# Oliverbansk/Holistic-Robot-Pose-Estimation

Hardware: AMD Instinct MI355X
Metric: images/sec/GPU fwd+bwd HRNet-W32 256x256 bs=64; 1/2/4/8-GPU scaling (higher is better)
Workload: dtype bf16; 1 GPU; full network (HRNet-W32 reg backbone + HRNet-W32 DepthNet + heads + FK loss) fwd+loss+bwd+clip+Adam, BASELINE.json configs[2]; global_batch=64, per_gpu_batch=64, image=3x256x256, hrnet_w32_passes_per_image=2, parallelism=dp1, backend=single-process, rccl_ranks=1, hip_graph=True, plan_mode=hybrid, inputs=resident in HBM, optimizer=hrpe_amd.optim.FusedClipAdam (clip 5 + Adam, lr 1e-4)

## Files before the change

### holistic-robot-pose-estimation_amd/csrc/conv_batch.h

```cpp
#pragma once
#include "conv_row.h"
#include <string.h>

namespace hrp {

struct ConvProblem {
  hrp_conv_desc d;
  ConvTiling t;
  int cfg;
  int pgrid;
  int pad[2];
  RowPlan r;
};

template <typename T, int NT, bool LIGHT>
__global__ __launch_bounds__(256, LIGHT ? 1 : 2) void conv_batch_kernel(const ConvProblem* __restrict__ tab, const BatchHdr h) {
  int base;
  const int g = batch_find(h, blockIdx.x, base);
  const ConvProblem& P = tab[g];
  const int bid = (int)blockIdx.x - base;
  const int slot = blockIdx.x & (HRP_STAT_SLOTS - 1);
  if constexpr (LIGHT) {
    switch (P.cfg) {
      case 0: conv_tile_body<T, 1, 2, 1, 4, NT, false, true>(P.d, P.t, bid, 1, slot); break;
      case 1: conv_tile_body<T, 1, 1, 1, 4, NT, false, true>(P.d, P.t, bid, 1, slot); break;
      default:
        if constexpr (NT == 9) conv_tile_body<T, 1, 2, 1, 4, NT, true, true>(P.d, P.t, bid, P.pgrid, slot);
        break;
    }
  } else {
    switch (P.cfg) {
      case 0: conv_tile_body<T, 1, 2, 1, 4, NT, false, true>(P.d, P.t, bid, 1, slot); break;
      case 1: conv_tile_body<T, 1, 1, 1, 4, NT, false, true>(P.d, P.t, bid, 1, slot); break;
      case 2: conv_tile_body<T, 2, 2, 1, 4, NT, false, true>(P.d, P.t, bid, 1, slot); break;
      case 5: if constexpr (NT == 9 && Elem<T>::SZ == 2) conv_row_body<32>(P.d, P.r, bid, slot); break;
      case 6: if constexpr (NT == 9 && Elem<T>::SZ == 2) conv_row_body<64>(P.d, P.r, bid, slot); break;
      case 7: if constexpr (NT == 9 && Elem<T>::SZ == 2) conv_deep_body<128>(P.d, P.r, bid, slot); break;
      case 8: if constexpr (NT == 9 && Elem<T>::SZ == 2) conv_deep_body<256>(P.d, P.r, bid, slot); break;
      case 9: if constexpr (NT == 9 && Elem<T>::SZ == 2) conv_img_body<128>(P.d, P.r, bid, slot); break;
      case 10: if constexpr (NT == 9 && Elem<T>::SZ == 2) conv_img_body<256>(P.d, P.r, bid, slot); break;
      default: conv_tile_body<T, 2, 1, 1, 4, NT, false, true>(P.d, P.t, bid, 1, slot); break;
    }
  }
}

template <typename T, int NT>
static int conv_batch_plan_one(const hrp_conv_desc& d, ConvProblem& P, int& lds) {
  int rc = -100;
  if constexpr (NT == 9 && Elem<T>::SZ == 2) {
    const int rc_ = hrp_conv_rowstrip_channels(&d);
    if (rc_) {
      row_plan(d, P.r);
      P.t = ConvTiling{};
      P.t.nblocks = row_grid(P.r, rc_);
      P.cfg = rc_ == 32 ? 5 : rc_ == 64 ? 6 : rc_ == 128 ? 7 : 8;
      if (P.r.img) P.cfg += 2;
      lds = row_lds_bytes(rc_, P.r.img);
      return HRP_OK;
    }
  }
  static const int budget_kb = 76;
  g_conv_lds_budget_kb = budget_kb;
  if (d.Cout <= 32) {
    rc = plan_cfg<T, 1, 2, 1, 4, NT>(d, P.t, lds, false); P.cfg = 0;
    if (rc == -100) { rc = plan_cfg<T, 1, 1, 1, 4, NT>(d, P.t, lds, false); P.cfg = 1; }
  } else {
    rc = plan_cfg<T, 2, 2, 1, 4, NT>(d, P.t, lds, false); P.cfg = 2;
    if (rc == -100) { rc = plan_cfg<T, 2, 1, 1, 4, NT>(d, P.t, lds, false); P.cfg = 3; }
    if (rc == -100) { rc = plan_cfg<T, 1, 2, 1, 4, NT>(d, P.t, lds, false); P.cfg = 0; }
    if (rc == -100) { rc = plan_cfg<T, 1, 1, 1, 4, NT>(d, P.t, lds, false); P.cfg = 1; }
  }
  if (rc == -100) {
    set_error("conv batch: no tile configuration fits LDS and the tap halo (H=%d W=%d Cin=%d stride=%d taps=%d)", d.H, d.W, d.Cin, d.in_stride, d.ntaps);
    return HRP_ERR_ARG;
  }
  return rc;
}

template <typename T, int NT>
static int conv_batch_prepare_nt(const hrp_conv_desc* descs, int n, ConvProblem* tab, hrp_batch_info* info) {
  constexpr int SZ = Elem<T>::SZ;
  ConvProblem probs[HRP_BATCH_MAX];
  long weight[HRP_BATCH_MAX];
  int lds_max = 0;
  for (int i = 0; i < n; ++i) {
    const hrp_conv_desc& d = descs[i];
    HRP_REQUIRE((d.Cin * SZ) % ROW == 0, "conv batch: Cin * sizeof(T) must be a multiple of 32 bytes (Cin=%d)", d.Cin);
    memset(&probs[i], 0, sizeof(ConvProblem));
    probs[i].d = d;
    int lds = 0;
    const int rc = conv_batch_plan_one<T, NT>(d, probs[i], lds);
    if (rc != HRP_OK) return rc;
    lds_max = lds > lds_max ? lds : lds_max;
    const int ct = probs[i].cfg >= 2 ? 2 : 1, pt = (probs[i].cfg & 1) ? 1 : 2;
    weight[i] = (long)cdiv(d.Cin * SZ, ROW) * NT * ct * pt;
    if (probs[i].cfg >= 5) weight[i] = (long)cdiv(d.Cin * SZ, ROW) * NT * (probs[i].cfg == 9 ? 8 : 4);
  }
  int order[HRP_BATCH_MAX];
  for (int i = 0; i < n; ++i) order[i] = i;
  for (int i = 1; i < n; ++i)
    for (int j = i; j > 0 && weight[order[j]] > weight[order[j - 1]]; --j) { int t_ = order[j]; order[j] = order[j - 1]; order[j - 1] = t_; }
  bool light = true;
  for (int i = 0; i < n; ++i) light = light && probs[i].cfg <= 1;
  static const int pwgs = 512;
  const int pcap = light && pwgs > 0 ? (pwgs / n < 32 ? 32 : pwgs / n) : 0;
  int blk = 0;
  for (int k = 0; k < n; ++k) {
    ConvProblem& P = probs[order[k]];
    info->blk0[k] = blk;
    if (NT == 9 && pcap > 0 && P.cfg == 0 && P.t.nblocks >= 2 * pcap && P.d.Cin * SZ <= 2 * ROW && !P.d.bnb_x) {
      P.cfg = 4;
      P.pgrid = pcap;
      blk += pcap;
    } else {
      blk += P.t.nblocks;
    }
    if (tab) tab[k] = P;
  }
  info->blk0[n] = blk;
  info->grid = blk;
  info->lds_bytes = lds_max;
  info->variant = NT + (light ? 100 : 0);
  return HRP_OK;
}

template <typename T>
static int conv_batch_prepare_t(const hrp_conv_desc* descs, int n, void* table, hrp_batch_info* info) {
  for (int i = 0; i < n; ++i) {
    const int rc = conv_check(&descs[i]);
    if (rc != HRP_OK) return rc;
    HRP_REQUIRE(descs[i].ntaps == descs[0].ntaps && descs[i].dtype == descs[0].dtype, "conv batch: mixed tap counts / element types");
    HRP_REQUIRE(descs[i].ntaps != 1 || !descs[i].bnb_x || (descs[i].bnb_mask && descs[i].bnb_consts && !descs[i].res),
                "conv batch: a 1x1 problem with a mask-less / residual epilogue reduce must be launched on its own (hrp_conv_pointwise)");
    HRP_REQUIRE(!(descs[i].dtype == HRP_F32 && descs[i].H == 1 && descs[i].W == 1 && descs[i].Cin >= 512),
                "conv batch: linear layers are launched one by one");
  }
  ConvProblem* tab = (ConvProblem*)table;
  switch (descs[0].ntaps) {
    case 1: return conv_batch_prepare_nt<T, 1>(descs, n, tab, info);
    case 2: return conv_batch_prepare_nt<T, 2>(descs, n, tab, info);
    case 4: return conv_batch_prepare_nt<T, 4>(descs, n, tab, info);
    case 9: return conv_batch_prepare_nt<T, 9>(descs, n, tab, info);
    default:
      set_error("conv batch: ntaps=%d is not one of the batched tap counts (1, 2, 4, 9)", descs[0].ntaps);
      return HRP_ERR_ARG;
  }
}

template <typename T, int NT, bool LIGHT>
static int conv_batch_launch_nt(const void* table_dev, const hrp_batch_info* info, hipStream_t s) {
  static bool attr_set = false;
  if (!attr_set) {
    (void)hipFuncSetAttribute((const void*)conv_batch_kernel<T, NT, LIGHT>, hipFuncAttributeMaxDynamicSharedMemorySize, 160 * 1024);
    attr_set = true;
  }
  const BatchHdr h = make_hdr(info->blk0, info->n);
  hipLaunchKernelGGL((conv_batch_kernel<T, NT, LIGHT>), dim3(info->grid), dim3(256), info->lds_bytes, s, (const ConvProblem*)table_dev, h);
  return check_launch("conv_batch_kernel");
}

template <typename T>
static int conv_batch_launch_t(const void* table_dev, const hrp_batch_info* info, hipStream_t s) {
  switch (info->variant) {
    case 1: return conv_batch_launch_nt<T, 1, false>(table_dev, info, s);
    case 2: return conv_batch_launch_nt<T, 2, false>(table_dev, info, s);
    case 4: return conv_batch_launch_nt<T, 4, false>(table_dev, info, s);
    case 9: return conv_batch_launch_nt<T, 9, false>(table_dev, info, s);
    case 101: return conv_batch_launch_nt<T, 1, true>(table_dev, info, s);
    case 102: return conv_batch_launch_nt<T, 2, true>(table_dev, info, s);
    case 104: return conv_batch_launch_nt<T, 4, true>(table_dev, info, s);
    case 109: return conv_batch_launch_nt<T, 9, true>(table_dev, info, s);
    default: set_error("conv batch: bad variant %d", info->variant); return HRP_ERR_ARG;
  }
}

}
```

### holistic-robot-pose-estimation_amd/csrc/conv_row.h

```cpp
#pragma once
#include "conv_tile.h"
#include <type_traits>

namespace hrp {

template <int C>
struct RowCfg {
  static constexpr int W = 2048 / C;
  static constexpr int P = 2 * C;
  static constexpr int S = P / 16;
  static constexpr int KS = C / 16;
  static constexpr int MT = C / 32;
  static constexpr int NCOL = W / 32;
  static constexpr int TH = 8;
  static constexpr int PXP = 1024 / P;
  static constexpr int ROWB = (W + 1) * P;
  static constexpr int NROWS = TH + 2;
  static constexpr int TILE_BYTES = P + NROWS * ROWB;
  static constexpr int CTAB_OFF = (TILE_BYTES + 255) & ~255;
  static constexpr int STAT_OFF = CTAB_OFF + 10 * C * 4;
  static constexpr bool PERSIST = C == 32;
  static constexpr int WLDS_OFF = STAT_OFF + 4 * 64 * 4;
  static constexpr int LDS_BYTES = WLDS_OFF + (PERSIST ? 9 * KS * 1024 : 0);
  static_assert(MT * NCOL == 2, "two waves side by side (columns or channel tiles), two on top of each other");
  __device__ static __forceinline__ int g(int x) { return C == 32 ? (x >> 2) & 3 : (x >> 1) & 7; }
};

struct RowPlan {
  int wslot[9];
  int nstrips, spi;
  FastDiv fd_spi;
  int img;
  int spw;
};

__device__ __forceinline__ void row_bn_consts(const double* stats, const float* gamma, const float* beta, float count, float eps,
                                              int c, int C, float& mean, float& inv, float& sc, float& sh) {
  const float m = slot_sum(stats, c, 2 * C) / count;
  const float var = fmaxf(slot_sum(stats, C + c, 2 * C) / count - m * m, 0.f);
  inv = rsqrtf(var + eps);
  mean = m;
  sc = gamma[c] * inv;
  sh = beta[c] - m * sc;
}

__device__ __forceinline__ float row_bn_act(float x, float sc, float sh) { return fmaf(x, sc, sh); }

static inline int row_channels(const hrp_conv_desc& d) {
  if (d.dtype != HRP_BF16 || d.ntaps != 9 || d.in_stride != 1 || d.out_stride != 1) return 0;
  if (d.Cin != d.Cout || (d.Cin != 32 && d.Cin != 64 && d.Cin != 128 && d.Cin != 256)) return 0;
  const int C = d.Cin;
  if (d.W != 2048 / C || d.Wo != d.W || d.Ho != d.H || d.H % 8 || d.y_H != d.Ho || d.y_W != d.Wo) return 0;
  if (d.x_pitch != C || d.y_pitch != C || d.w_cout_pad != C || (d.res && d.res_pitch != C)) return 0;
  if (((uintptr_t)d.x | (uintptr_t)d.y | (uintptr_t)d.w | (uintptr_t)d.res) % 16) return 0;
  if (d.bias) return 0;
  if (d.bnb_x && (d.bnb_x_pitch != C || !d.bnb_stats || !d.bnb_gamma || !d.bnb_beta || !d.stats ||
                  d.relu || d.scale || (uintptr_t)d.bnb_x % 16)) return 0;
  if (d.bnb_x && d.bnb_mask && (d.bnb_mask_pitch != C / 8 || (uintptr_t)d.bnb_mask % 2)) return 0;
  if (d.pro_mode < 0 || d.pro_mode > 3) return 0;
  if (d.pro_mode && (!d.pro_stats || !d.pro_gamma || !d.pro_beta)) return 0;
  if (d.pro_mode == 2 && (!d.pro_x2 || !d.pro_bsums || (uintptr_t)d.pro_x2 % 16)) return 0;
  if (d.pro_mode == 3 && (!d.pro_x2 || (uintptr_t)d.pro_x2 % 16 || !d.pro_side || !d.pro_mask || d.pro_side2)) return 0;
  if (d.pro_mode < 2 && (d.pro_mask || d.pro_side2)) return 0;
  if ((d.pro_side && (uintptr_t)d.pro_side % 16) || (d.pro_side2 && (uintptr_t)d.pro_side2 % 16)) return 0;
  if (d.res_mask && (!d.res || (uintptr_t)d.res_mask % 2 || d.relu || d.scale)) return 0;
  if ((long long)d.N * d.H * d.W * C * 2 >= (1ll << 31)) return 0;
  unsigned seen = 0;
  for (int i = 0; i < 9; ++i) {
    if (d.dy[i] < -1 || d.dy[i] > 1 || d.dx[i] < -1 || d.dx[i] > 1) return 0;
    seen |= 1u << ((d.dy[i] + 1) * 3 + d.dx[i] + 1);
  }
  return seen == 0x1ff ? C : 0;
}

static inline void row_plan(const hrp_conv_desc& d, RowPlan& rp) {
  for (int i = 0; i < 9; ++i) rp.wslot[(d.dy[i] + 1) * 3 + d.dx[i] + 1] = d.wtap[i];
  rp.spi = d.H / 8;
  rp.nstrips = d.N * rp.spi;
  rp.fd_spi = make_fastdiv(rp.spi);
  rp.img = 0;
  rp.spw = rp.nstrips >= 256 ? 2 : 1;
  if (rp.spi % rp.spw || d.Cin != 32) rp.spw = 1;
  static const bool no_img = false;
  if (!no_img && (d.Cin == 128 || d.Cin == 256) && d.H == d.W) {
    rp.img = 1;
    rp.nstrips = d.Cin == 128 ? d.N : ((d.N + 1) / 2) * 2;
  }
}


__device__ __forceinline__ float row_keep_if_bit(const float v, const int bits, const int i) {
  const int m = (int)((unsigned)bits << (31 - i)) >> 31;
  return __int_as_float(__float_as_int(v) & m);
}

struct RowPro {
  float sc[8], sh[8], c1[8], c0[8];
  __device__ __forceinline__ void load(const float* ctab, const int C, const int cb) {
#pragma unroll
    for (int i = 0; i < 8; i += 4) {
      const float4 va = *(const float4*)(ctab + cb + i), vb = *(const float4*)(ctab + C + cb + i);
      sc[i] = va.x; sc[i + 1] = va.y; sc[i + 2] = va.z; sc[i + 3] = va.w;
      sh[i] = vb.x; sh[i + 1] = vb.y; sh[i + 2] = vb.z; sh[i + 3] = vb.w;
    }
  }
  __device__ __forceinline__ void load2(const float* ctab, const int C, const int cb) {
#pragma unroll
    for (int i = 0; i < 8; i += 4) {
      const float4 va = *(const float4*)(ctab + 2 * C + cb + i), vb = *(const float4*)(ctab + 3 * C + cb + i);
      const float4 v0 = *(const float4*)(ctab + 4 * C + cb + i), v1 = *(const float4*)(ctab + 5 * C + cb + i);
      const float a[4] = {va.x, va.y, va.z, va.w}, b[4] = {vb.x, vb.y, vb.z, vb.w};
      const float k0[4] = {v0.x, v0.y, v0.z, v0.w}, k1[4] = {v1.x, v1.y, v1.z, v1.w};
#pragma unroll
      for (int e = 0; e < 4; ++e) {
        c1[i + e] = -sc[i + e] * k1[e] * a[e];
        c0[i + e] = -sc[i + e] * fmaf(k1[e], b[e], k0[e]);
      }
    }
  }
  __device__ __forceinline__ uint4 act(const uint4 raw) const {
    float f[8];
    Elem<bf16_t>::unpack(raw, f);
#pragma unroll
    for (int i = 0; i < 8; ++i) f[i] = fmaxf(row_bn_act(f[i], sc[i], sh[i]), 0.f);
    return Elem<bf16_t>::pack(f);
  }
  __device__ __forceinline__ uint4 fwd3(const uint4 raw, const uint4 res, unsigned& bits) const {
    float f[8], r[8];
    Elem<bf16_t>::unpack(raw, f);
    Elem<bf16_t>::unpack(res, r);
    bits = 0;
#pragma unroll
    for (int i = 0; i < 8; ++i) {
      f[i] = fmaxf(row_bn_act(f[i], sc[i], sh[i]) + r[i], 0.f);
      bits |= (f[i] > 0.f ? 1u : 0u) << i;
    }
    return Elem<bf16_t>::pack(f);
  }
  template <bool BITS, bool GM>
  __device__ __forceinline__ uint4 bwd_t(const uint4 graw, const uint4 xraw, const int bits, uint4& gm) const {
    float gq[8], xv[8];
    Elem<bf16_t>::unpack(graw, gq);
    Elem<bf16_t>::unpack(xraw, xv);
#pragma unroll
    for (int i = 0; i < 8; ++i) {
      if constexpr (BITS) gq[i] = row_keep_if_bit(gq[i], bits, i);
      else gq[i] = row_bn_act(xv[i], sc[i], sh[i]) > 0.f ? gq[i] : 0.f;
    }
    if constexpr (GM) gm = Elem<bf16_t>::pack(gq);
#pragma unroll
    for (int i = 0; i < 8; ++i) gq[i] = fmaf(sc[i], gq[i], fmaf(c1[i], xv[i], c0[i]));
    return Elem<bf16_t>::pack(gq);
  }
  template <bool EXT>
  __device__ __forceinline__ uint4 bwd(const uint4 graw, const uint4 xraw, const int bits, uint4& gm, const bool ub, const bool wgm) const {
    if constexpr (!EXT) return bwd_t<false, false>(graw, xraw, bits, gm);
    else {
      if (ub) return wgm ? bwd_t<true, true>(graw, xraw, bits, gm) : bwd_t<true, false>(graw, xraw, bits, gm);
      return wgm ? bwd_t<false, true>(graw, xraw, bits, gm) : bwd_t<false, false>(graw, xraw, bits, gm);
    }
  }
};

__device__ __forceinline__ void row_side2(const hrp_conv_desc& d, const unsigned off, const uint4 gm) {
  char* q = (char*)d.pro_side2 + off;
// ... 120 lines not shown
  if (aff) {
#pragma unroll
    for (int i = 0; i < 16; i += 4) {
      const float4 a = *(const float4*)(d.scale + cl + i), b = *(const float4*)(d.shift + cl + i);
      sc[i] = a.x; sc[i + 1] = a.y; sc[i + 2] = a.z; sc[i + 3] = a.w;
      sh[i] = b.x; sh[i + 1] = b.y; sh[i + 2] = b.z; sh[i + 3] = b.w;
    }
  }
#pragma unroll
  for (int t = 0; t < NT; ++t) {
#pragma unroll
    for (int hh = 0; hh < 2; ++hh) {
      float v[8];
#pragma unroll
      for (int i = 0; i < 8; ++i) v[i] = acc[t][8 * hh + i];
      if (aff) {
#pragma unroll
        for (int i = 0; i < 8; ++i) v[i] = v[i] * sc[8 * hh + i] + sh[8 * hh + i];
      }
      if (rg_) {
        float r[8];
        Elem<bf16_t>::unpack(rr[t][hh], r);
        if constexpr (EXT) {
          if (d.res_mask && ((okmask >> t) & 1)) {
            const int rb = d.res_mask[(off[t] >> 4) + hh];
#pragma unroll
            for (int i = 0; i < 8; ++i) r[i] = row_keep_if_bit(r[i], rb, i);
          }
        }
#pragma unroll
        for (int i = 0; i < 8; ++i) v[i] += r[i];
      }
      if (d.relu) {
#pragma unroll
        for (int i = 0; i < 8; ++i) v[i] = fmaxf(v[i], 0.f);
      }
      const uint4 pk = Elem<bf16_t>::pack(v);
      if ((okmask >> t) & 1) *(uint4*)(yg + off[t] + 16 * hh) = pk;
      if (STATS && d.stats && ((okmask >> t) & 1)) {
        Elem<bf16_t>::unpack(pk, v);
#pragma unroll
        for (int i = 0; i < 8; ++i) { s1[8 * hh + i] += v[i]; s2[8 * hh + i] = fmaf(v[i], v[i], s2[8 * hh + i]); }
      }
    }
  }
}

__device__ __forceinline__ float row_reduce32(const float (&s1)[16], const float (&s2)[16], const int l31) {
  float v16[16], v8[8], v4[4], v2[2];
  {
    const bool up = (l31 & 16) != 0;
#pragma unroll
    for (int j = 0; j < 16; ++j) { const float keep = up ? s2[j] : s1[j], send = up ? s1[j] : s2[j]; v16[j] = keep + __shfl_xor(send, 16, 64); }
  }
  {
    const bool up = (l31 & 8) != 0;
#pragma unroll
    for (int j = 0; j < 8; ++j) { const float keep = up ? v16[8 + j] : v16[j], send = up ? v16[j] : v16[8 + j]; v8[j] = keep + __shfl_xor(send, 8, 64); }
  }
  {
    const bool up = (l31 & 4) != 0;
#pragma unroll
    for (int j = 0; j < 4; ++j) { const float keep = up ? v8[4 + j] : v8[j], send = up ? v8[j] : v8[4 + j]; v4[j] = keep + __shfl_xor(send, 4, 64); }
  }
  {
    const bool up = (l31 & 2) != 0;
#pragma unroll
    for (int j = 0; j < 2; ++j) { const float keep = up ? v4[2 + j] : v4[j], send = up ? v4[j] : v4[2 + j]; v2[j] = keep + __shfl_xor(send, 2, 64); }
  }
  const bool up = (l31 & 1) != 0;
  const float keep = up ? v2[1] : v2[0], send = up ? v2[0] : v2[1];
  return keep + __shfl_xor(send, 1, 64);
}

__device__ __forceinline__ void row_stats_commit(const hrp_conv_desc& d, const float v1, const int l31, const int cl, const float* ctab,
                                                 const int C, const bool bnb, const int stat_slot) {
  const int which = l31 >> 4, c = cl + (l31 & 15);
  const float other = __shfl_xor(v1, 16, 64);
  float tot = v1;
  if (bnb && which == 1) tot = fmaf(ctab[6 * C + c], v1, ctab[7 * C + c] * other);
  atomicAdd(d.stats + stat_slot * 2 * C + which * C + c, (double)tot);
}

template <int C, bool EXT>
__device__ __forceinline__ void conv_row_body_t(const hrp_conv_desc& d, const RowPlan& rp, int bid, const int stat_slot) {
  using R = RowCfg<C>;
  constexpr int W = R::W, P = R::P, S = R::S, KS = R::KS, TH = R::TH, ROWB = R::ROWB, NROWS = R::NROWS;
  extern __shared__ __attribute__((aligned(16))) char smem[];
  float* ctab = (float*)(smem + R::CTAB_OFF);
  float* stat_lds = (float*)(smem + R::STAT_OFF);

  const int tid = threadIdx.x, lane = tid & 63;
  const int wave = __builtin_amdgcn_readfirstlane(tid >> 6);
  const int l31 = lane & 31, half = lane >> 5;
  const int sel = wave & 1, rg = wave >> 1;
  const int col = R::NCOL == 2 ? sel : 0;
  const int m = R::MT == 2 ? sel : 0;
  HRP_CSTAMP(0);

  const int ngroups = (rp.nstrips + rp.spw - 1) / rp.spw;
  if ((ngroups & 7) == 0) bid = (bid & 7) * (ngroups >> 3) + (bid >> 3);
  const int s_begin = bid * rp.spw, s_end = min(s_begin + rp.spw, rp.nstrips);
  const int H = d.H;
  const int pro = d.pro_mode;
  const bool ub = EXT && d.pro_mask != nullptr, wgm = EXT && d.pro_side2 != nullptr;

  bf16x8 wf[9][KS];
  const int co_lane = m * 32 + 16 * ((l31 >> 2) & 1) + 4 * (l31 >> 3) + (l31 & 3);
  const char* wl = (const char*)d.w + co_lane * ROW + half * 16;
  char* wlds = smem + R::WLDS_OFF;
  if constexpr (R::PERSIST) {
#pragma unroll
    for (int f = 0; f < 9 * KS; ++f)
      if ((f & 3) == wave) dma16(wl + (size_t)(((f % KS) * d.w_ntaps + rp.wslot[f / KS]) * C) * ROW, wlds + f * 1024);
  } else {
#pragma unroll
    for (int t = 0; t < 9; ++t)
#pragma unroll
      for (int kk = 0; kk < KS; ++kk)
        wf[t][kk] = *(const bf16x8*)(wl + (size_t)((kk * d.w_ntaps + rp.wslot[t]) * C) * ROW);
  }

  const int px_in_piece = lane / S;
  const int xcol = wave * R::PXP + px_in_piece;
  const int lslot = (lane % S) ^ R::g(xcol);
  const unsigned lane_off = (unsigned)(wave * 1024 + px_in_piece * P + lslot * 16);
  char* lds_rows = smem + P;
  auto strip_of = [&](int s, int& n, int& y0) { n = fdiv(s, rp.fd_spi); y0 = (s - n * rp.spi) * TH; };
  auto stage = [&](int s) {
    int n, y0;
    strip_of(s, n, y0);
    const char* xg = (const char*)d.x + (unsigned)n * (unsigned)(H * W * P) + lane_off;
#pragma unroll
    for (int rs = 0; rs < NROWS; ++rs) {
      const int y = y0 - 1 + rs;
      char* dst = lds_rows + rs * ROWB + wave * 1024;
      if (y >= 0 && y < H) dma16(xg + y * (W * P), dst);
      else *(uint4*)(dst + lane * 16) = make_uint4(0, 0, 0, 0);
    }
  };
  stage(s_begin);
  if (tid < (NROWS + 1) * S) {
    const int k = tid / S, j = tid - k * S;
    *(uint4*)(smem + (k == 0 ? 0 : P + (k - 1) * ROWB + W * P) + j * 16) = make_uint4(0, 0, 0, 0);
  }

  const bool bnb = d.bnb_x != nullptr;
  if (pro != 0 && tid < C) {
    float mean, inv, sc, sh;
    row_bn_consts(d.pro_stats, d.pro_gamma, d.pro_beta, d.pro_count, d.pro_eps, tid, C, mean, inv, sc, sh);
    ctab[0 * C + tid] = sc; ctab[1 * C + tid] = sh;
    if (pro == 2) {
      ctab[2 * C + tid] = inv; ctab[3 * C + tid] = -mean * inv;
      ctab[4 * C + tid] = slot_sum(d.pro_bsums, tid, 2 * C) / d.pro_count;
      ctab[5 * C + tid] = slot_sum(d.pro_bsums, C + tid, 2 * C) / d.pro_count;
    }
  }
  if (bnb && tid >= 64 && tid < 64 + C) {
    const int c = tid - 64;
    float mean, inv, sc, sh;
    row_bn_consts(d.bnb_stats, d.bnb_gamma, d.bnb_beta, d.bnb_count, d.bnb_eps, c, C, mean, inv, sc, sh);
    ctab[8 * C + c] = sc; ctab[9 * C + c] = sh;
    ctab[6 * C + c] = inv; ctab[7 * C + c] = -mean * inv;
  }
  HRP_CSTAMP(1);
  if (pro != 0) __syncthreads();

  int baddr[3][KS];
#pragma unroll
  for (int dxi = 0; dxi < 3; ++dxi) {
    const int xq = col * 32 + l31 + dxi - 1;
#pragma unroll
    for (int kk = 0; kk < KS; ++kk)
      baddr[dxi][kk] = P + rg * 4 * ROWB + xq * P + (((2 * kk + half) ^ R::g(xq)) << 4);
  }
  const int cl = m * 32 + 16 * half;
  float vtot = 0.f;

  const int s_stop = R::PERSIST ? s_end : s_begin + 1;
  for (int s = s_begin; s < s_stop; ++s) {
    int n, y0;
    strip_of(s, n, y0);
    const unsigned img_off = (unsigned)n * (unsigned)(H * W * P);
    asm volatile("s_waitcnt vmcnt(0)" ::: "memory");
    if (pro != 0) {
      RowPro pc;
      int cb = lslot * 8;
      asm volatile("" : "+v"(cb));
      pc.load(ctab, C, cb);
      char* side = (char*)d.pro_side;
      if (pro == 1) {
#pragma unroll
        for (int rs = 0; rs < NROWS; ++rs) {
          const int y = y0 - 1 + rs;
          if (y < 0 || y >= H) continue;
          char* p = lds_rows + rs * ROWB + wave * 1024 + lane * 16;
          const uint4 o = pc.act(*(const uint4*)p);
          *(uint4*)p = o;
          if (side && rs >= 1 && rs <= TH) *(uint4*)(side + img_off + lane_off + y * (W * P)) = o;
        }
      } else {
        const bool f3 = EXT && pro == 3;
        if (!f3) pc.load2(ctab, C, cb);
        const char* x2g = (const char*)d.pro_x2 + img_off + lane_off;
        const uint8_t* mg = (EXT && d.pro_mask) ? d.pro_mask + ((img_off + lane_off) >> 4) : nullptr;
#pragma unroll
        for (int r0 = 0; r0 < NROWS; r0 += 5) {
          uint4 x2[5];
          int bits[5];
#pragma unroll
          for (int j = 0; j < 5; ++j) {
            const int y = y0 - 1 + r0 + j;
            x2[j] = make_uint4(0, 0, 0, 0);
            bits[j] = -1;
            if (y >= 0 && y < H) {
              x2[j] = *(const uint4*)(x2g + y * (W * P));
              if constexpr (EXT) {
                if (mg && !f3) bits[j] = mg[y * (W * P / 16)];
              }
            }
          }
#pragma unroll
          for (int j = 0; j < 5; ++j) {
            const int rs = r0 + j, y = y0 - 1 + rs;
            if (y < 0 || y >= H) continue;
            char* p = lds_rows + rs * ROWB + wave * 1024 + lane * 16;
            if constexpr (EXT) {
              if (f3) {
                unsigned ob;
                const uint4 o3 = pc.fwd3(*(const uint4*)p, x2[j], ob);
                *(uint4*)p = o3;
                if (rs >= 1 && rs <= TH) {
                  *(uint4*)(side + img_off + lane_off + y * (W * P)) = o3;
                  const_cast<uint8_t*>(mg)[y * (W * P / 16)] = (uint8_t)ob;
                }
                continue;
              }
            }
            uint4 gm;
            const uint4 o = pc.template bwd<EXT>(*(const uint4*)p, x2[j], bits[j], gm, ub, wgm);
            *(uint4*)p = o;
            if (rs >= 1 && rs <= TH) {
              const unsigned off = img_off + lane_off + y * (W * P);
              if (side) *(uint4*)(side + off) = o;
              if constexpr (EXT) {
                if (d.pro_side2) row_side2(d, off, gm);
              }
            }
          }
        }
      }
    }
    __syncthreads();
    if (s == s_begin) HRP_CSTAMP(2);
    if constexpr (R::PERSIST) {
#pragma unroll
      for (int f = 0; f < 9 * KS; ++f) wf[f / KS][f % KS] = *(const bf16x8*)(wlds + f * 1024 + lane * 16);
    }

    f32x16 acc[4];
#pragma unroll
    for (int o = 0; o < 4; ++o)
#pragma unroll
      for (int i = 0; i < 16; ++i) acc[o][i] = 0.f;
    {
      constexpr int NSTEP = 6 * 3 * KS, RING = 4, AHEAD = 3;
      bf16x8 bq[RING];
      auto rd = [&](int q) -> bf16x8 {
        const int irel = q / (3 * KS), dxi = (q / KS) % 3, kk = q % KS;
        return *(const bf16x8*)(smem + baddr[dxi][kk] + irel * ROWB);
      };
#pragma unroll
      for (int q = 0; q < AHEAD; ++q) bq[q % RING] = rd(q);
#pragma unroll
      for (int q = 0; q < NSTEP; ++q) {
        if (q + AHEAD < NSTEP) bq[(q + AHEAD) % RING] = rd(q + AHEAD);
        const int irel = q / (3 * KS), dxi = (q / KS) % 3, kk = q % KS;
#pragma unroll
        for (int o = 0; o < 4; ++o) {
          const int dyi = irel - o;
          if (dyi >= 0 && dyi <= 2)
            acc[o] = __builtin_amdgcn_mfma_f32_32x32x16_bf16(wf[dyi * 3 + dxi][kk], bq[q % RING], acc[o], 0, 0, 0);
        }
        __builtin_amdgcn_sched_barrier(0);
      }
    }
    if (s == s_begin) HRP_CSTAMP(4);
    if constexpr (R::PERSIST) {
      if (s + 1 < s_end) {
        __syncthreads();
        stage(s + 1);
      }
    }

    float s1[16], s2[16];
#pragma unroll
    for (int i = 0; i < 16; ++i) s1[i] = s2[i] = 0.f;
    {
      const unsigned out_off = img_off + (unsigned)((y0 + rg * 4) * W + col * 32 + l31) * P + cl * 2;
      constexpr int EG = EXT ? 2 : 4;
#pragma unroll
      for (int o0 = 0; o0 < 4; o0 += EG) {
        unsigned off[EG];
#pragma unroll
        for (int o = 0; o < EG; ++o) off[o] = out_off + (o0 + o) * (W * P);
        if constexpr (EG == 4) row_epilogue<4, EXT>(d, acc, off, 0xfu, cl, ctab, C, bnb, s1, s2);
        else row_epilogue<EG, EXT>(d, *(const f32x16(*)[EG])&acc[o0], off, (1u << EG) - 1, cl, ctab, C, bnb, s1, s2);
      }
    }
    if (d.stats) vtot += row_reduce32(s1, s2, l31);
    if (s == s_begin) HRP_CSTAMP(5);
  }
  if (d.stats) {
    stat_lds[wave * 64 + lane] = vtot;
    __syncthreads();
    if (tid < 2 * C) {
      const int which = tid / C, c = tid - which * C;
      const int mc = c >> 5, hq = (c >> 4) & 1, j = c & 15;
      auto tot = [&](int wh) {
        const int li = hq * 32 + wh * 16 + j;
        float t = 0.f;
        if (R::MT == 1) t = (stat_lds[0 * 64 + li] + stat_lds[1 * 64 + li]) + (stat_lds[2 * 64 + li] + stat_lds[3 * 64 + li]);
        else t = stat_lds[mc * 64 + li] + stat_lds[(mc + 2) * 64 + li];
        return t;
      };
      float t = tot(which);
      if (bnb && which == 1) t = fmaf(ctab[6 * C + c], t, ctab[7 * C + c] * tot(0));
      atomicAdd(d.stats + stat_slot * 2 * C + which * C + c, (double)t);
    }
  }
  HRP_CSTAMP(6);
  HRP_CSTAMP(7);
}

template <int C>
__device__ __forceinline__ void conv_row_body(const hrp_conv_desc& d, const RowPlan& rp, const int bid, const int stat_slot) {
  if (row_ext(d)) conv_row_body_t<C, true>(d, rp, bid, stat_slot);
  else conv_row_body_t<C, false>(d, rp, bid, stat_slot);
}

template <int C>
__global__ __launch_bounds__(256, 2) void conv_row_kernel(const hrp_conv_desc d, const RowPlan rp) {
  conv_row_body<C>(d, rp, blockIdx.x, blockIdx.x & (HRP_STAT_SLOTS - 1));
}


template <int C>
struct DeepCfg {
  static constexpr int W = 2048 / C;
  static constexpr int P = 2 * C;
  static constexpr int S = P / 16;
  static constexpr int KS = C / 16;
  static constexpr int PXP = 1024 / P;
  static constexpr int ROWB = (W + 1) * P;
  static constexpr int TH = 8, NROWS = TH + 2;
  static constexpr int MW = C == 128 ? 1 : 2, NW = 4 / MW;
  static constexpr int RPT = 32 / W;
  static constexpr int TILE_BYTES = P + NROWS * ROWB;
  static constexpr int CTAB_OFF = (TILE_BYTES + 255) & ~255;
  static constexpr int LDS_BYTES = CTAB_OFF + 10 * C * 4;
  static_assert(NW * RPT == TH, "the wave's tiles cover the strip");
  __device__ static __forceinline__ int f(int y, int x) { return (y * W + x) & 15; }
};

template <int C, bool EXT>
__device__ __forceinline__ void conv_deep_body_t(const hrp_conv_desc& d, const RowPlan& rp, int bid, const int stat_slot) {
  using R = DeepCfg<C>;
  constexpr int W = R::W, P = R::P, S = R::S, KS = R::KS, TH = R::TH, ROWB = R::ROWB, NROWS = R::NROWS;
  constexpr int MW = R::MW, NW = R::NW, RPT = R::RPT;
  extern __shared__ __attribute__((aligned(16))) char smem[];
  float* ctab = (float*)(smem + R::CTAB_OFF);

  const int tid = threadIdx.x, lane = tid & 63;
  const int wave = __builtin_amdgcn_readfirstlane(tid >> 6);
  const int l31 = lane & 31, half = lane >> 5;
  HRP_CSTAMP(0);
  if ((rp.nstrips & 7) == 0) bid = (bid & 7) * (rp.nstrips >> 3) + (bid >> 3);
  const int n = fdiv(bid, rp.fd_spi);
  const int y0 = (bid - n * rp.spi) * TH;
  const int H = d.H;
  const int pro = d.pro_mode;
  const bool ub = EXT && d.pro_mask != nullptr, wgm = EXT && d.pro_side2 != nullptr;
  const unsigned img_off = (unsigned)n * (unsigned)(H * W * P);
  char* lds_rows = smem + P;

  const int px_in_piece = lane / S, pslot = lane % S;
  const int xcol = wave * R::PXP + px_in_piece;
  auto lane_off_of = [&](int y) { return (unsigned)(wave * 1024 + px_in_piece * P + ((pslot ^ R::f(y, xcol)) << 4)); };
  {
    const char* xg = (const char*)d.x + img_off;
#pragma unroll
    for (int rs = 0; rs < NROWS; ++rs) {
// ... 390 lines not shown
    auto rd = [&](int kkoff, int q) -> bf16x8 {
      const int tap = q / NT, t = q % NT;
      const int dyi = tap / 3, dxi = tap % 3;
      const int b = (dyi == 0 && t % TPI == 0) ? Bt[dxi] : (dyi == 2 && t % TPI == TPI - 1) ? Bb[dxi] : Bm[tap];
      return *(const bf16x8*)(smem + (b ^ kkoff) + t * T);
    };
    auto chunk = [&](int kk, auto uc) {
      constexpr int u = decltype(uc)::value;
      const int kkoff = kk << 5;
      const bool more = kk + 1 < KS;
#pragma unroll
      for (int q = 0; q < CH; ++q) {
        constexpr int GS = GT * NT;
        const int gi = q / GS;
        if (q % GS == 0) {
          const int g = kk * NG + gi;
          if constexpr (C == 128) wload(g + 2, wbuf[(gi + 2) % 3], (gi + 2) % 3);
          else wload(g + 1, wbuf[(u + 1) & 1], 0);
        }
        if (q + AHEAD < CH) bq[(q + AHEAD) % RING] = rd(kkoff, q + AHEAD);
        else if (more) bq[(q + AHEAD) % RING] = rd(kkoff + 32, q + AHEAD - CH);
        const int bi = C == 128 ? gi : u;
        acc[q % NT] = __builtin_amdgcn_mfma_f32_32x32x16_bf16(wbuf[bi][(q / NT) % GT], bq[q % RING], acc[q % NT], 0, 0, 0);
        __builtin_amdgcn_sched_barrier(0);
      }
    };
#pragma unroll
    for (int g = 0; g < NBUF - 1; ++g) wload(g, wbuf[g], g % NG);
#pragma unroll
    for (int q = 0; q < AHEAD; ++q) bq[q % RING] = rd(0, q);
    for (int kk = 0; kk < KS; kk += 2) {
      chunk(kk, std::integral_constant<int, 0>{});
      chunk(kk + 1, std::integral_constant<int, 1>{});
    }
  }
  HRP_CSTAMP(4);

  {
    const int cl = cbk * 128 + wave * 32 + 16 * half;
    const unsigned pix0 = grp_off + (unsigned)l31 * P + cl * 2;
    float s1[16], s2[16];
#pragma unroll
    for (int i = 0; i < 16; ++i) s1[i] = s2[i] = 0.f;
    constexpr int EG = NT == 8 ? 2 : 4;
#pragma unroll
    for (int t0 = 0; t0 < NT; t0 += EG) {
      unsigned off[EG];
#pragma unroll
      for (int t = 0; t < EG; ++t) off[t] = pix0 + (unsigned)(t0 + t) * (32 * P);
      row_epilogue<EG, EXT>(d, *(const f32x16(*)[EG])&acc[t0], off, (okmask >> t0) & ((1u << EG) - 1), cl, ctab, C, bnb, s1, s2);
    }
    if (d.stats) row_stats_commit(d, row_reduce32(s1, s2, l31), l31, cl, ctab, C, bnb, stat_slot);
  }
  HRP_CSTAMP(6);
  HRP_CSTAMP(7);
}

template <int C>
__device__ __forceinline__ void conv_img_body(const hrp_conv_desc& d, const RowPlan& rp, const int bid, const int stat_slot) {
  if (row_ext(d)) conv_img_body_t<C, true>(d, rp, bid, stat_slot);
  else conv_img_body_t<C, false>(d, rp, bid, stat_slot);
}

template <int C>
__global__ __launch_bounds__(256, 2) void conv_img_kernel(const hrp_conv_desc d, const RowPlan rp) {
  conv_img_body<C>(d, rp, blockIdx.x, blockIdx.x & (HRP_STAT_SLOTS - 1));
}

static inline int row_grid(const RowPlan& rp, int C) {
  return (C <= 64 && !rp.img) ? (rp.nstrips + rp.spw - 1) / rp.spw : rp.nstrips;
}

static inline int row_lds_bytes(int C, int img) {
  if (img) return C == 128 ? ImgCfg<128>::LDS_BYTES : ImgCfg<256>::LDS_BYTES;
  return C == 32 ? RowCfg<32>::LDS_BYTES : C == 64 ? RowCfg<64>::LDS_BYTES : C == 128 ? DeepCfg<128>::LDS_BYTES : DeepCfg<256>::LDS_BYTES;
}

static int launch_conv_row(const hrp_conv_desc& d, hipStream_t s) {
  const int C = row_channels(d);
  if (!C) return -100;
  RowPlan rp;
  row_plan(d, rp);
  if (rp.img && C == 128) { rp.img = 0; rp.nstrips = d.N * rp.spi; }
  if (C == 32) hipLaunchKernelGGL(conv_row_kernel<32>, dim3(row_grid(rp, 32)), dim3(256), RowCfg<32>::LDS_BYTES, s, d, rp);
  else if (C == 64) hipLaunchKernelGGL(conv_row_kernel<64>, dim3(row_grid(rp, 64)), dim3(256), RowCfg<64>::LDS_BYTES, s, d, rp);
  else if (rp.img) {
    static bool attr = false;
    if (!attr) {
      (void)hipFuncSetAttribute((const void*)conv_img_kernel<128>, hipFuncAttributeMaxDynamicSharedMemorySize, 160 * 1024);
      (void)hipFuncSetAttribute((const void*)conv_img_kernel<256>, hipFuncAttributeMaxDynamicSharedMemorySize, 160 * 1024);
      attr = true;
    }
    if (C == 128) hipLaunchKernelGGL(conv_img_kernel<128>, dim3(rp.nstrips), dim3(256), ImgCfg<128>::LDS_BYTES, s, d, rp);
    else hipLaunchKernelGGL(conv_img_kernel<256>, dim3(rp.nstrips), dim3(256), ImgCfg<256>::LDS_BYTES, s, d, rp);
  }
  else if (C == 128) hipLaunchKernelGGL(conv_deep_kernel<128>, dim3(rp.nstrips), dim3(256), DeepCfg<128>::LDS_BYTES, s, d, rp);
  else {
    static bool attr = false;
    if (!attr) { (void)hipFuncSetAttribute((const void*)conv_deep_kernel<256>, hipFuncAttributeMaxDynamicSharedMemorySize, 160 * 1024); attr = true; }
    hipLaunchKernelGGL(conv_deep_kernel<256>, dim3(rp.nstrips), dim3(256), DeepCfg<256>::LDS_BYTES, s, d, rp);
  }
  return check_launch("conv_row_kernel");
}

}
```

Baseline: 2055 images/sec.

## Halve row-conv strip height, persist all row strips, prefetch epilogue and prologue operands

The 3x3 row-strip convolution for 32/64 channels now uses 4-row strips instead of 8, and every workgroup processes several strips persistently. The strips-per-workgroup count is sized against a fixed slot budget, both in standalone launches and in batched launches where it is shared with the other problems. Prologue second-input rows and mask bits are DMA'd into LDS during staging, and the next strip's staging now overlaps the current epilogue. Epilogue residual/mask loads are issued before the MFMA loop for C=32, and non-parked weights are reloaded per strip. This is meant to improve load balance and hide global-memory latency, at the cost of more halo rows, extra LDS and more register pressure.

```diff
diff --git a/holistic-robot-pose-estimation_amd/csrc/conv_batch.h b/holistic-robot-pose-estimation_amd/csrc/conv_batch.h
--- a/holistic-robot-pose-estimation_amd/csrc/conv_batch.h
+++ b/holistic-robot-pose-estimation_amd/csrc/conv_batch.h
@@ -96,6 +96,24 @@
     weight[i] = (long)cdiv(d.Cin * SZ, ROW) * NT * ct * pt;
     if (probs[i].cfg >= 5) weight[i] = (long)cdiv(d.Cin * SZ, ROW) * NT * (probs[i].cfg == 9 ? 8 : 4);
   }
+  {
+    long strips = 0, others = 0;
+    for (int i = 0; i < n; ++i) {
+      if (probs[i].cfg == 5 || probs[i].cfg == 6) strips += probs[i].r.nstrips;
+      else others += probs[i].t.nblocks;
+    }
+    if (strips) {
+      const long free_slots = ROW_SLOTS - others > ROW_SLOTS / 4 ? ROW_SLOTS - others : ROW_SLOTS / 4;
+      int spw = (int)((strips + free_slots - 1) / free_slots);
+      if (spw < 2) spw = 2;
+      for (int i = 0; i < n; ++i) {
+        if (probs[i].cfg != 5 && probs[i].cfg != 6) continue;
+        probs[i].r.spw = spw;
+        probs[i].t.nblocks = row_grid(probs[i].r, probs[i].d.Cin);
+        weight[i] = (long)cdiv(probs[i].d.Cin * SZ, ROW) * NT * RowCfg<32>::RPW * spw;
+      }
+    }
+  }
   int order[HRP_BATCH_MAX];
   for (int i = 0; i < n; ++i) order[i] = i;
   for (int i = 1; i < n; ++i)
diff --git a/holistic-robot-pose-estimation_amd/csrc/conv_row.h b/holistic-robot-pose-estimation_amd/csrc/conv_row.h
--- a/holistic-robot-pose-estimation_amd/csrc/conv_row.h
+++ b/holistic-robot-pose-estimation_amd/csrc/conv_row.h
@@ -3,6 +3,10 @@
 #include <type_traits>
 
 namespace hrp {
+
+#ifndef HRP_ROW_EPI_EARLY
+#define HRP_ROW_EPI_EARLY(C, EXT) ((C) == 32)
+#endif
 
 template <int C>
 struct RowCfg {
@@ -12,17 +16,20 @@
   static constexpr int KS = C / 16;
   static constexpr int MT = C / 32;
   static constexpr int NCOL = W / 32;
-  static constexpr int TH = 8;
+  static constexpr int TH = 4;
+  static constexpr int RPW = TH / 2;
   static constexpr int PXP = 1024 / P;
   static constexpr int ROWB = (W + 1) * P;
   static constexpr int NROWS = TH + 2;
   static constexpr int TILE_BYTES = P + NROWS * ROWB;
-  static constexpr int CTAB_OFF = (TILE_BYTES + 255) & ~255;
+  static constexpr int X2_OFF = (TILE_BYTES + 255) & ~255;
+  static constexpr int CTAB_OFF = X2_OFF + NROWS * 4096;
   static constexpr int STAT_OFF = CTAB_OFF + 10 * C * 4;
-  static constexpr bool PERSIST = C == 32;
+  static constexpr bool PARK = C == 32;
   static constexpr int WLDS_OFF = STAT_OFF + 4 * 64 * 4;
-  static constexpr int LDS_BYTES = WLDS_OFF + (PERSIST ? 9 * KS * 1024 : 0);
+  static constexpr int LDS_BYTES = WLDS_OFF + (PARK ? 9 * KS * 1024 : 0);
   static_assert(MT * NCOL == 2, "two waves side by side (columns or channel tiles), two on top of each other");
+  static_assert(2 * LDS_BYTES <= 160 * 1024, "two workgroups per CU");
   __device__ static __forceinline__ int g(int x) { return C == 32 ? (x >> 2) & 3 : (x >> 1) & 7; }
 };
 
@@ -73,14 +80,23 @@
   return seen == 0x1ff ? C : 0;
 }
 
+static constexpr int ROW_SLOTS = 512;
+
+static inline void row_set_slots(RowPlan& rp, int slots) {
+  if (slots < 1) slots = 1;
+  rp.spw = (rp.nstrips + slots - 1) / slots;
+  if (rp.spw < 2) rp.spw = 2;
+}
+
 static inline void row_plan(const hrp_conv_desc& d, RowPlan& rp) {
   for (int i = 0; i < 9; ++i) rp.wslot[(d.dy[i] + 1) * 3 + d.dx[i] + 1] = d.wtap[i];
-  rp.spi = d.H / 8;
+  const bool deep = d.Cin > 64;
+  rp.spi = deep ? d.H / 8 : d.H / RowCfg<32>::TH;
   rp.nstrips = d.N * rp.spi;
   rp.fd_spi = make_fastdiv(rp.spi);
   rp.img = 0;
-  rp.spw = rp.nstrips >= 256 ? 2 : 1;
-  if (rp.spi % rp.spw || d.Cin != 32) rp.spw = 1;
+  rp.spw = 1;
+  if (!deep) row_set_slots(rp, ROW_SLOTS);
   static const bool no_img = false;
   if (!no_img && (d.Cin == 128 || d.Cin == 256) && d.H == d.W) {
     rp.img = 1;
@@ -367,10 +383,108 @@
   atomicAdd(d.stats + stat_slot * 2 * C + which * C + c, (double)tot);
 }
 
+template <int NT, bool EXT>
+__device__ __forceinline__ void row_epi_prefetch(const hrp_conv_desc& d, const unsigned (&off)[NT], const unsigned okmask, const bool bnb,
+                                                 RowEpiOps<NT>& e) {
+  if (bnb) {
+    if constexpr (!EXT) row_epi_load<NT, true, false, false>(d, off, okmask, e);
+    else {
+      const bool ubits = d.bnb_mask != nullptr, ures = d.res != nullptr;
+      if (ubits) { if (ures) row_epi_load<NT, true, true, true>(d, off, okmask, e); else row_epi_load<NT, true, true, false>(d, off, okmask, e); }
+      else { if (ures) row_epi_load<NT, true, false, true>(d, off, okmask, e); else row_epi_load<NT, true, false, false>(d, off, okmask, e); }
+    }
+  } else if (d.res) {
+    row_epi_load<NT, false, false, true>(d, off, okmask, e);
+  } else {
+#pragma unroll
+    for (int t = 0; t < NT; ++t) {
+      e.xr[t][0] = e.xr[t][1] = e.rr[t][0] = e.rr[t][1] = make_uint4(0, 0, 0, 0);
+      e.mb[t] = 0;
+      e.rb[t] = 0xffff;
+    }
+  }
+}
+
+template <int NT>
+__device__ __forceinline__ void row_epi_landed(RowEpiOps<NT>& e) {
+#pragma unroll
+  for (int t = 0; t < NT; ++t) {
+#pragma unroll
+    for (int hh = 0; hh < 2; ++hh) {
+      asm volatile("" : "+v"(e.xr[t][hh].x), "+v"(e.xr[t][hh].y), "+v"(e.xr[t][hh].z), "+v"(e.xr[t][hh].w));
+      asm volatile("" : "+v"(e.rr[t][hh].x), "+v"(e.rr[t][hh].y), "+v"(e.rr[t][hh].z), "+v"(e.rr[t][hh].w));
+    }
+    asm volatile("" : "+v"(e.mb[t]), "+v"(e.rb[t]));
+  }
+}
+
+template <int NT, bool EXT>
+__device__ __forceinline__ void row_epilogue_ops(const hrp_conv_desc& d, const f32x16 (&acc)[NT], const unsigned (&off)[NT],
+                                                 const unsigned okmask, const int cl, const float* ctab, const int C, const bool bnb,
+                                                 const RowEpiOps<NT>& e, float (&s1)[16], float (&s2)[16]) {
+  char* yg = (char*)d.y;
+  if (bnb) {
+    if constexpr (!EXT) row_epi_bnb_math<NT, false, false>(d, acc, off, okmask, cl, ctab, C, e, s1, s2);
+    else {
+      const bool ubits = d.bnb_mask != nullptr, ures = d.res != nullptr;
+      if (ubits) { if (ures) row_epi_bnb_math<NT, true, true>(d, acc, off, okmask, cl, ctab, C, e, s1, s2); else row_epi_bnb_math<NT, true, false>(d, acc, off, okmask, cl, ctab, C, e, s1, s2); }
+      else { if (ures) row_epi_bnb_math<NT, false, true>(d, acc, off, okmask, cl, ctab, C, e, s1, s2); else row_epi_bnb_math<NT, false, false>(d, acc, off, okmask, cl, ctab, C, e, s1, s2); }
+    }
+    return;
+  }
+  const bool ures = d.res != nullptr;
+  float sc[16], sh[16];
+  const bool aff = d.scale != nullptr;
+  if (aff) {
+#pragma unroll
+    for (int i = 0; i < 16; i += 4) {
+      const float4 a = *(const float4*)(d.scale + cl + i), b = *(const float4*)(d.shift + cl + i);
+      sc[i] = a.x; sc[i + 1] = a.y; sc[i + 2] = a.z; sc[i + 3] = a.w;
+      sh[i] = b.x; sh[i + 1] = b.y; sh[i + 2] = b.z; sh[i + 3] = b.w;
+    }
+  }
+#pragma unroll
+  for (int t = 0; t < NT; ++t) {
+#pragma unroll
+    for (int hh = 0; hh < 2; ++hh) {
+      float v[8];
+#pragma unroll
+      for (int i = 0; i < 8; ++i) v[i] = acc[t][8 * hh + i];
+      if (aff) {
+#pragma unroll
+        for (int i = 0; i < 8; ++i) v[i] = v[i] * sc[8 * hh + i] + sh[8 * hh + i];
+      }
+      if (ures) {
+        float r[8];
+        Elem<bf16_t>::unpack(e.rr[t][hh], r);
+        if constexpr (EXT) {
+          if (d.res_mask) {
+#pragma unroll
+            for (int i = 0; i < 8; ++i) r[i] = row_keep_if_bit(r[i], e.rb[t], 8 * hh + i);
+          }
+        }
+#pragma unroll
+        for (int i = 0; i < 8; ++i) v[i] += r[i];
+      }
+      if (d.relu) {
+#pragma unroll
+        for (int i = 0; i < 8; ++i) v[i] = fmaxf(v[i], 0.f);
+      }
+      const uint4 pk = Elem<bf16_t>::pack(v);
+      if ((okmask >> t) & 1) *(uint4*)(yg + off[t] + 16 * hh) = pk;
+      if (d.stats && ((okmask >> t) & 1)) {
+        Elem<bf16_t>::unpack(pk, v);
+#pragma unroll
+        for (int i = 0; i < 8; ++i) { s1[8 * hh + i] += v[i]; s2[8 * hh + i] = fmaf(v[i], v[i], s2[8 * hh + i]); }
+      }
+    }
+  }
+}
+
 template <int C, bool EXT>
 __device__ __forceinline__ void conv_row_body_t(const hrp_conv_desc& d, const RowPlan& rp, int bid, const int stat_slot) {
   using R = RowCfg<C>;
-  constexpr int W = R::W, P = R::P, S = R::S, KS = R::KS, TH = R::TH, ROWB = R::ROWB, NROWS = R::NROWS;
+  constexpr int W = R::W, P = R::P, S = R::S, KS = R::KS, TH = R::TH, RPW = R::RPW, ROWB = R::ROWB, NROWS = R::NROWS;
   extern __shared__ __attribute__((aligned(16))) char smem[];
   float* ctab = (float*)(smem + R::CTAB_OFF);
   float* stat_lds = (float*)(smem + R::STAT_OFF);
@@ -388,40 +502,59 @@
   const int s_begin = bid * rp.spw, s_end = min(s_begin + rp.spw, rp.nstrips);
   const int H = d.H;
   const int pro = d.pro_mode;
-  const bool ub = EXT && d.pro_mask != nullptr, wgm = EXT && d.pro_side2 != nullptr;
+  const bool ub = EXT && pro == 2 && d.pro_mask != nullptr, wgm = EXT && d.pro_side2 != nullptr;
 
   bf16x8 wf[9][KS];
   const int co_lane = m * 32 + 16 * ((l31 >> 2) & 1) + 4 * (l31 >> 3) + (l31 & 3);
   const char* wl = (const char*)d.w + co_lane * ROW + half * 16;
   char* wlds = smem + R::WLDS_OFF;
-  if constexpr (R::PERSIST) {
+  if constexpr (R::PARK) {
 #pragma unroll
     for (int f = 0; f < 9 * KS; ++f)
       if ((f & 3) == wave) dma16(wl + (size_t)(((f % KS) * d.w_ntaps + rp.wslot[f / KS]) * C) * ROW, wlds + f * 1024);
-  } else {
-#pragma unroll
-    for (int t = 0; t < 9; ++t)
-#pragma unroll
-      for (int kk = 0; kk < KS; ++kk)
-        wf[t][kk] = *(const bf16x8*)(wl + (size_t)((kk * d.w_ntaps + rp.wslot[t]) * C) * ROW);
   }
 
   const int px_in_piece = lane / S;
   const int xcol = wave * R::PXP + px_in_piece;
   const int lslot = (lane % S) ^ R::g(xcol);
-  const unsigned lane_off = (unsigned)(wave * 1024 + px_in_piece * P + lslot * 16);
+  const unsigned lane_off0 = (unsigned)(wave * 1024 + px_in_piece * P + lslot * 16);
   char* lds_rows = smem + P;
+  char* lds_x2 = smem + R::X2_OFF;
+  int mbits[NROWS];
+#pragma unroll
+  for (int rs = 0; rs < NROWS; ++rs) mbits[rs] = -1;
   auto strip_of = [&](int s, int& n, int& y0) { n = fdiv(s, rp.fd_spi); y0 = (s - n * rp.spi) * TH; };
   auto stage = [&](int s) {
     int n, y0;
     strip_of(s, n, y0);
-    const char* xg = (const char*)d.x + (unsigned)n * (unsigned)(H * W * P) + lane_off;
+    const unsigned img_off = (unsigned)n * (unsigned)(H * W * P);
+    unsigned lane_off = lane_off0;
+    asm volatile("" : "+v"(lane_off));
+    const char* xg = (const char*)d.x + img_off + lane_off;
 #pragma unroll
     for (int rs = 0; rs < NROWS; ++rs) {
       const int y = y0 - 1 + rs;
       char* dst = lds_rows + rs * ROWB + wave * 1024;
       if (y >= 0 && y < H) dma16(xg + y * (W * P), dst);
       else *(uint4*)(dst + lane * 16) = make_uint4(0, 0, 0, 0);
+    }
+    if (pro >= 2) {
+      const char* x2g = (const char*)d.pro_x2 + img_off + lane_off;
+#pragma unroll
+      for (int rs = 0; rs < NROWS; ++rs) {
+        const int y = y0 - 1 + rs;
+        if (y >= 0 && y < H) dma16(x2g + y * (W * P), lds_x2 + rs * 4096 + wave * 1024);
+      }
+      if constexpr (EXT) {
+        if (ub) {
+          const uint8_t* mg = d.pro_mask + ((img_off + lane_off) >> 4);
+#pragma unroll
+          for (int rs = 0; rs < NROWS; ++rs) {
+            const int y = y0 - 1 + rs;
+            if (y >= 0 && y < H) mbits[rs] = mg[y * (W * P / 16)];
+          }
+        }
+      }
     }
   };
   stage(s_begin);
@@ -457,16 +590,17 @@
     const int xq = col * 32 + l31 + dxi - 1;
 #pragma unroll
     for (int kk = 0; kk < KS; ++kk)
-      baddr[dxi][kk] = P + rg * 4 * ROWB + xq * P + (((2 * kk + half) ^ R::g(xq)) << 4);
+      baddr[dxi][kk] = P + rg * RPW * ROWB + xq * P + (((2 * kk + half) ^ R::g(xq)) << 4);
   }
   const int cl = m * 32 + 16 * half;
   float vtot = 0.f;
 
-  const int s_stop = R::PERSIST ? s_end : s_begin + 1;
-  for (int s = s_begin; s < s_stop; ++s) {
+  for (int s = s_begin; s < s_end; ++s) {
     int n, y0;
     strip_of(s, n, y0);
     const unsigned img_off = (unsigned)n * (unsigned)(H * W * P);
+    unsigned lane_off = lane_off0;
+    asm volatile("" : "+v"(lane_off));
     asm volatile("s_waitcnt vmcnt(0)" ::: "memory");
     if (pro != 0) {
       RowPro pc;
@@ -487,69 +621,70 @@
       } else {
         const bool f3 = EXT && pro == 3;
         if (!f3) pc.load2(ctab, C, cb);
-        const char* x2g = (const char*)d.pro_x2 + img_off + lane_off;
-        const uint8_t* mg = (EXT && d.pro_mask) ? d.pro_mask + ((img_off + lane_off) >> 4) : nullptr;
-#pragma unroll
-        for (int r0 = 0; r0 < NROWS; r0 += 5) {
-          uint4 x2[5];
-          int bits[5];
-#pragma unroll
-          for (int j = 0; j < 5; ++j) {
-            const int y = y0 - 1 + r0 + j;
-            x2[j] = make_uint4(0, 0, 0, 0);
-            bits[j] = -1;
-            if (y >= 0 && y < H) {
-              x2[j] = *(const uint4*)(x2g + y * (W * P));
-              if constexpr (EXT) {
-                if (mg && !f3) bits[j] = mg[y * (W * P / 16)];
+#pragma unroll
+        for (int rs = 0; rs < NROWS; ++rs) {
+          const int y = y0 - 1 + rs;
+          if (y < 0 || y >= H) continue;
+          char* p = lds_rows + rs * ROWB + wave * 1024 + lane * 16;
+          const uint4 x2 = *(const uint4*)(lds_x2 + rs * 4096 + wave * 1024 + lane * 16);
+          const unsigned off = img_off + lane_off + y * (W * P);
+          if constexpr (EXT) {
+            if (f3) {
+              unsigned ob;
+              const uint4 o3 = pc.fwd3(*(const uint4*)p, x2, ob);
+              *(uint4*)p = o3;
+              if (rs >= 1 && rs <= TH) {
+                *(uint4*)(side + off) = o3;
+                const_cast<uint8_t*>(d.pro_mask)[off >> 4] = (uint8_t)ob;
               }
+              continue;
             }
           }
-#pragma unroll
-          for (int j = 0; j < 5; ++j) {
-            const int rs = r0 + j, y = y0 - 1 + rs;
-            if (y < 0 || y >= H) continue;
-            char* p = lds_rows + rs * ROWB + wave * 1024 + lane * 16;
+          uint4 gm;
+          const uint4 o = pc.template bwd<EXT>(*(const uint4*)p, x2, mbits[rs], gm, ub, wgm);
+          *(uint4*)p = o;
+          if (rs >= 1 && rs <= TH) {
+            if (side) *(uint4*)(side + off) = o;
             if constexpr (EXT) {
-              if (f3) {
-                unsigned ob;
-                const uint4 o3 = pc.fwd3(*(const uint4*)p, x2[j], ob);
-                *(uint4*)p = o3;
-                if (rs >= 1 && rs <= TH) {
-                  *(uint4*)(side + img_off + lane_off + y * (W * P)) = o3;
-                  const_cast<uint8_t*>(mg)[y * (W * P / 16)] = (uint8_t)ob;
-                }
-                continue;
-              }
-            }
-            uint4 gm;
-            const uint4 o = pc.template bwd<EXT>(*(const uint4*)p, x2[j], bits[j], gm, ub, wgm);
-            *(uint4*)p = o;
-            if (rs >= 1 && rs <= TH) {
-              const unsigned off = img_off + lane_off + y * (W * P);
-              if (side) *(uint4*)(side + off) = o;
-              if constexpr (EXT) {
-                if (d.pro_side2) row_side2(d, off, gm);
-              }
+              if (d.pro_side2) row_side2(d, off, gm);
             }
           }
         }
       }
     }
+    if constexpr (!R::PARK) {
+      const char* wls = wl;
+      asm volatile("" : "+v"(wls));
+#pragma unroll
+      for (int t = 0; t < 9; ++t)
+#pragma unroll
+        for (int kk = 0; kk < KS; ++kk)
+          wf[t][kk] = *(const bf16x8*)(wls + (size_t)((kk * d.w_ntaps + rp.wslot[t]) * C) * ROW);
+    }
     __syncthreads();
     if (s == s_begin) HRP_CSTAMP(2);
-    if constexpr (R::PERSIST) {
+    if constexpr (R::PARK) {
 #pragma unroll
       for (int f = 0; f < 9 * KS; ++f) wf[f / KS][f % KS] = *(const bf16x8*)(wlds + f * 1024 + lane * 16);
     }
 
-    f32x16 acc[4];
-#pragma unroll
-    for (int o = 0; o < 4; ++o)
+    constexpr bool EARLY = HRP_ROW_EPI_EARLY(C, EXT);
+    unsigned off[RPW];
+    {
+      const unsigned out_off = img_off + (unsigned)((y0 + rg * RPW) * W + col * 32 + l31) * P + cl * 2;
+#pragma unroll
+      for (int o = 0; o < RPW; ++o) off[o] = out_off + o * (W * P);
+    }
+    RowEpiOps<RPW> eo;
+    if constexpr (EARLY) row_epi_prefetch<RPW, EXT>(d, off, (1u << RPW) - 1, bnb, eo);
+
+    f32x16 acc[RPW];
+#pragma unroll
+    for (int o = 0; o < RPW; ++o)
 #pragma unroll
       for (int i = 0; i < 16; ++i) acc[o][i] = 0.f;
     {
-      constexpr int NSTEP = 6 * 3 * KS, RING = 4, AHEAD = 3;
+      constexpr int NSTEP = (RPW + 2) * 3 * KS, RING = 4, AHEAD = 3;
       bf16x8 bq[RING];
       auto rd = [&](int q) -> bf16x8 {
         const int irel = q / (3 * KS), dxi = (q / KS) % 3, kk = q % KS;
@@ -562,7 +697,7 @@
         if (q + AHEAD < NSTEP) bq[(q + AHEAD) % RING] = rd(q + AHEAD);
         const int irel = q / (3 * KS), dxi = (q / KS) % 3, kk = q % KS;
 #pragma unroll
-        for (int o = 0; o < 4; ++o) {
+        for (int o = 0; o < RPW; ++o) {
           const int dyi = irel - o;
           if (dyi >= 0 && dyi <= 2)
             acc[o] = __builtin_amdgcn_mfma_f32_32x32x16_bf16(wf[dyi * 3 + dxi][kk], bq[q % RING], acc[o], 0, 0, 0);
@@ -571,28 +706,17 @@
       }
     }
     if (s == s_begin) HRP_CSTAMP(4);
-    if constexpr (R::PERSIST) {
-      if (s + 1 < s_end) {
-        __syncthreads();
-        stage(s + 1);
-      }
+    if constexpr (EARLY) row_epi_landed<RPW>(eo);
+    else row_epi_prefetch<RPW, EXT>(d, off, (1u << RPW) - 1, bnb, eo);
+    if (s + 1 < s_end) {
+      __syncthreads();
+      stage(s + 1);
     }
 
     float s1[16], s2[16];
 #pragma unroll
     for (int i = 0; i < 16; ++i) s1[i] = s2[i] = 0.f;
-    {
-      const unsigned out_off = img_off + (unsigned)((y0 + rg * 4) * W + col * 32 + l31) * P + cl * 2;
-      constexpr int EG = EXT ? 2 : 4;
-#pragma unroll
-      for (int o0 = 0; o0 < 4; o0 += EG) {
-        unsigned off[EG];
-#pragma unroll
-        for (int o = 0; o < EG; ++o) off[o] = out_off + (o0 + o) * (W * P);
-        if constexpr (EG == 4) row_epilogue<4, EXT>(d, acc, off, 0xfu, cl, ctab, C, bnb, s1, s2);
-        else row_epilogue<EG, EXT>(d, *(const f32x16(*)[EG])&acc[o0], off, (1u << EG) - 1, cl, ctab, C, bnb, s1, s2);
-      }
-    }
+    row_epilogue_ops<RPW, EXT>(d, acc, off, (1u << RPW) - 1, cl, ctab, C, bnb, eo, s1, s2);
     if (d.stats) vtot += row_reduce32(s1, s2, l31);
     if (s == s_begin) HRP_CSTAMP(5);
   }
@@ -1149,7 +1273,11 @@
   RowPlan rp;
   row_plan(d, rp);
   if (rp.img && C == 128) { rp.img = 0; rp.nstrips = d.N * rp.spi; }
-  if (C == 32) hipLaunchKernelGGL(conv_row_kernel<32>, dim3(row_grid(rp, 32)), dim3(256), RowCfg<32>::LDS_BYTES, s, d, rp);
+  if (C == 32) {
+    static bool attr = false;
+    if (!attr) { (void)hipFuncSetAttribute((const void*)conv_row_kernel<32>, hipFuncAttributeMaxDynamicSharedMemorySize, 160 * 1024); attr = true; }
+    hipLaunchKernelGGL(conv_row_kernel<32>, dim3(row_grid(rp, 32)), dim3(256), RowCfg<32>::LDS_BYTES, s, d, rp);
+  }
   else if (C == 64) hipLaunchKernelGGL(conv_row_kernel<64>, dim3(row_grid(rp, 64)), dim3(256), RowCfg<64>::LDS_BYTES, s, d, rp);
   else if (rp.img) {
     static bool attr = false;
```

New measurement: 2040 images/sec. No clear change (-0.7%).
